# AlbrechtL/welle.io

Measured on AMD Instinct MI355X. Metric: DAB Mode-I ensembles/s (x real-time), higher is better.
Workload: dtype f32 (FFT/demap) + u16 (Viterbi metrics) + u8 (GF(256))

## Files before the change

### welle.io_amd/csrc/dabphy_fused.hip

```cpp
#include "dabphy_internal.h"
#include "soft_layout.h"

namespace {

bool step_table(const std::vector<map_t>& m, int nsteps, int n_in, int rows, bool skew, std::vector<MscStep>& st, int& n_windows, int& why)
{
    const int PITCH = MSC_ROW_PITCH, SLOT = rows * MSC_ROW_PITCH, ZERO = 2 * SLOT;
    constexpr int PADDING = 6;
    st.assign((size_t)nsteps + PADDING, MscStep{0, 0});
    std::vector<int> wlo((size_t)nsteps, -1), whi((size_t)nsteps, -1);
    for (int q = 0; q < nsteps; q++) {
        uint32_t off[4];
        for (int j = 0; j < 4; j++) {
            const int u = map_index(m[4 * q + j]);
            if (u < 0) { off[j] = (uint32_t)ZERO; continue; }
            const int w = u >> 4, col = u & 15;
            off[j] = (uint32_t)((w & 1) * SLOT + (skew ? layout::tdi_row(col) : 0) * PITCH + col);
            if (wlo[q] < 0) wlo[q] = w;
            whi[q] = w;
        }
        st[q].off01 = off[0] | (off[1] << 16); st[q].off23 = off[2] | (off[3] << 16);
    }
    for (int q = nsteps; q < nsteps + PADDING; q++) st[(size_t)q].off01 = st[(size_t)q].off23 = (uint32_t)ZERO | ((uint32_t)ZERO << 16);
    n_windows = (n_in + 15) / 16;
    std::vector<int> low_after((size_t)nsteps, n_windows);
    for (int q = nsteps - 2, low = n_windows; q >= 0; q--) { if (wlo[q + 1] >= 0) low = wlo[q + 1]; low_after[q] = low; }
    int seen = 1, prev_low = 0;
    std::vector<int> load_step((size_t)n_windows + 2, -10);
    bool ok = nsteps % 6 == 0; why = ok ? 0 : 8;
    for (int q = 0; q < nsteps; q++) {
        if (whi[q] > seen) {
            st[q].off01 |= MSC_FIRST_USE; seen = whi[q];
            if (q - 1 - load_step[seen] < 2) { ok = false; why |= 1; }
        }
        if (whi[q] >= 0 && whi[q] - wlo[q] > 1) { ok = false; why |= 2; }
        if (low_after[q] > prev_low) {
            if (low_after[q] != prev_low + 1 && low_after[q] < n_windows) { ok = false; why |= 4; }
            prev_low = low_after[q];
            if (prev_low + 1 < n_windows) { st[q].off01 |= MSC_LOAD_NEXT; load_step[prev_low + 1] = q; }
        }
    }
    return ok;
}

}

extern "C" {

size_t soft_ens_stride(const dabphy_handle* h)
{
    return ((size_t)h->cfg.max_frames + 5 + 1) * SOFT_PER_FRAME;
}

int fused_class_tables(dabphy_handle* h, const dabphy_protection& prot, bool fic, DevBuf (&steps)[FUSED_VARIANTS], int (&n_windows)[FUSED_VARIANTS])
{
    const std::vector<map_t> m = depuncture_map(&prot);
    const int nsteps = prot.nbits + 6, n_in = protection_input_bits(&prot);
    for (int v = 0; v < FUSED_VARIANTS; v++) {
        std::vector<MscStep> st; int nw = 0, why = 0;
        const bool ok = step_table(m, nsteps, n_in, FUSED_ROWS[v], !fic, st, nw, why);
        if (!ok && debug_env("DABPHY_DEBUG")) fprintf(stderr, "dabphy: class nbits %d: no fused decode (window schedule, reason %d)\n", prot.nbits, why);
        n_windows[v] = ok ? nw : 0;
        int r;
        if ((r = ensure(h, steps[v], st.size() * sizeof(MscStep)))) return r;
        HIPCHK(h, hipMemcpy(steps[v].p, st.data(), st.size() * sizeof(MscStep), hipMemcpyHostToDevice));
    }
    return DABPHY_OK;
}

int dabphy_test_fused_windows(const dabphy_protection* prot, int32_t n_windows[FUSED_VARIANTS])
{
    if (!prot || !n_windows || !protection_valid(prot) || prot->nbits > PRBS_MAX_BITS) return DABPHY_ERR_INVALID;
    dabphy_protection pf; protection_fic(&pf);
    const bool fic = !memcmp(prot, &pf, sizeof pf);
    const std::vector<map_t> m = depuncture_map(prot);
    for (int v = 0; v < FUSED_VARIANTS; v++) {
        std::vector<MscStep> st; int nw = 0, why = 0;
        n_windows[v] = step_table(m, prot->nbits + 6, protection_input_bits(prot), FUSED_ROWS[v], !fic, st, nw, why) ? nw : 0;
    }
    return DABPHY_OK;
}

}

namespace {
bool sp_kernel_takes(int nsteps) { return nsteps % 6 == 0 && nsteps <= SP_MAXSTEPS[SP_VARIANTS - 1]; }
bool sp_wanted(const dabphy_handle* h, uint64_t n_cw) { return h->fused_msc && h->cfg.decode_shape != 1 && (h->cfg.decode_shape >= 2 || (h->sp_max_codewords > 0 && n_cw <= h->sp_max_codewords)); }
struct Draft {
    uint32_t F = 0; bool want_fic = false; int v = 0;
    uint64_t total_cw = 0; bool use_sp = false;
    std::vector<FusedClass> cls; std::vector<int> idx; bool fic_in = false; size_t max_steps = 0;
    std::vector<uint32_t> work, item_off; uint64_t item_rows = 0;
    bool sp_two = false, tb_split = false, dec_by_item = false; int n_slots = 0; size_t slot_cells = 0, dec_cells = 0;
};

void choose_shape(const dabphy_handle* h, Draft& D)
{
    const bool fic = D.want_fic && h->fused_fic;
    D.total_cw = (uint64_t)h->cfg.n_ensembles * D.F * 4 * (fic ? 1 : 0);
    size_t longest = fic ? 774 : 0; bool takes = true;
    for (auto& c : h->classes) { D.total_cw += (uint64_t)4 * D.F * c.pairs.size(); longest = std::max(longest, (size_t)c.prot.nbits + 6); takes = takes && sp_kernel_takes(c.prot.nbits + 6); }
    const bool scratch_below_a_gib = D.total_cw * (uint64_t)hist_cells(longest, false) * sizeof(uint2) <= ((uint64_t)1 << 30);
    D.use_sp = takes && sp_wanted(h, D.total_cw) && (h->cfg.decode_shape >= 2 || scratch_below_a_gib);
}
void admit_classes(const dabphy_handle* h, Draft& D)
{
    const int nseg = (FUSED_ROWS[D.v] - 64) / 15, F = (int)D.F;
    auto reach_ok = [&](int n_ens_spanned) { return (uint64_t)n_ens_spanned * soft_ens_stride(h) <= 0xffffffffull; };
    auto ens_span = [&](const std::vector<MscPair>& pr) {
        int span = 1;
        for (size_t p = 0; p < pr.size(); p++) span = std::max(span, pr[std::min(pr.size() - 1, p + (size_t)nseg - 1)].ens - pr[p].ens + 1);
        return span;
    };
    for (size_t i = 0; i < h->classes.size(); i++) {
        const auto& c = h->classes[i];
        if (h->fused_msc && (D.use_sp || (c.n_windows[D.v] > 0 && reach_ok(ens_span(c.pairs))))) { D.cls.push_back(msc_fused_class(c, D.F, D.v)); D.idx.push_back((int)i); }
    }
    D.fic_in = D.want_fic && h->fused_fic && (D.use_sp || (h->fic_windows[D.v] > 0 && reach_ok((16 + F - 1) / F + 1)));
    if (D.fic_in) D.cls.push_back(fic_fused_class(h, h->s_fib.as<uint8_t>(), (int)(h->cfg.n_ensembles * D.F * 4), D.v));
    for (const FusedClass& fc : D.cls) D.max_steps = std::max(D.max_steps, (size_t)fc.nsteps);
}
int build_work_list(dabphy_handle* h, Draft& D)
{
    if (D.cls.size() > WORK_MAX_CLASSES) { h->err = "more than 255 protection classes"; return DABPHY_ERR_INVALID; }
    struct Item { int nsteps, ci, n_groups; }; std::vector<Item> items;
    for (size_t ci = 0; ci < D.cls.size(); ci++) items.push_back({D.cls[ci].nsteps, (int)ci, (D.cls[ci].n_cw + 63) / 64});
    std::stable_sort(items.begin(), items.end(), [](const Item& a, const Item& b) { return a.nsteps > b.nsteps; });
    for (const Item& it : items) {
        if (it.n_groups > (int)WORK_MAX_GROUPS) { h->err = "class too large for the fused decode's work list"; return DABPHY_ERR_INVALID; }
        for (int g = 0; g < it.n_groups; g++) { D.work.push_back(work_item((uint32_t)it.ci, (uint32_t)g)); D.item_off.push_back((uint32_t)D.item_rows); D.item_rows += (uint64_t)it.nsteps; }
    }
    return DABPHY_OK;
}
void lay_out_scratch(const dabphy_handle* h, Draft& D)
{
    const int slots = fused_wave_slots(D.v);
    D.sp_two = D.use_sp && sp_two_for(h, D.total_cw);
    D.n_slots = D.use_sp ? (int)D.work.size() * (D.sp_two ? 32 : 64) : (int)std::min<size_t>(D.work.size(), (size_t)slots);
    D.slot_cells = D.use_sp ? hist_cells(D.max_steps, D.sp_two) : D.max_steps * 64;
    D.tb_split = h->tb_split && !D.use_sp && D.item_rows < 0xffffffffull && !D.work.empty();
    D.dec_by_item = !D.use_sp && (D.tb_split || debug_env("DABPHY_FORCE_DEC_BY_ITEM") || D.item_rows < (uint64_t)D.n_slots * D.max_steps) && D.item_rows < 0xffffffffull;
    D.dec_cells = D.dec_by_item ? (size_t)D.item_rows * 64 : (size_t)D.n_slots * D.slot_cells;
}
int reserve_buffers(dabphy_handle* h, const Draft& D)
{
    int r;
    if (D.work.empty()) return DABPHY_OK;
    if ((r = ensure(h, h->vdec, D.dec_cells * sizeof(uint2))) || (D.dec_by_item && (r = ensure(h, h->fused_dec_off, D.item_off.size() * sizeof(uint32_t))))) return r;
    if (D.tb_split && (r = ensure(h, h->fused_done, (D.work.size() + 2) * sizeof(uint32_t)))) return r;
    if (D.tb_split && !h->tb_stream && ((r = new_stream(h, &h->tb_stream)) || (r = new_event(h, &h->ev_tb_fork)) || (r = new_event(h, &h->ev_tb_join)))) return r;
    if ((r = ensure(h, h->fused_cls, D.cls.size() * sizeof(FusedClass))) || (r = ensure(h, h->fused_work, D.work.size() * sizeof(uint32_t)))) return r;
    return h->d_fused_next ? DABPHY_OK : device_block(h, &h->d_fused_next, 1);
}
int upload_changed(dabphy_handle* h, const Draft& D)
{
    auto& P = h->fplan;
    const bool in_place = P.valid && P.buf_gen == h->buf_gen;
    const bool same_cls = in_place && table_holds(P.host_cls, D.cls);
    const bool same_work = in_place && table_holds(P.host_work, D.work) && P.dec_by_item == D.dec_by_item;
    if (P.valid && (!same_cls || !same_work)) HIPCHK(h, hipStreamSynchronize(h->stream));
    int r = same_cls ? 0 : upload_kept(h, h->fused_cls, P.host_cls, D.cls);
    if (!r && !same_work) r = upload_kept(h, h->fused_work, P.host_work, D.work);
    if (!r && !same_work && D.dec_by_item) r = upload_kept(h, h->fused_dec_off, P.host_dec_off, D.item_off);
    return r;
}
void keep_plan(dabphy_handle* h, const Draft& D)
{
    auto& P = h->fplan;
    if (debug_env("DABPHY_DEBUG")) fprintf(stderr, "dabphy: decode plan for %u frames per call: %s, %zu of %zu classes%s, %zu groups, %d work-groups, decision scratch %s\n", D.F, D.use_sp ? (D.sp_two ? "state-parallel, two code words per wavefront" : "state-parallel") : "lane-per-code-word", D.idx.size(), h->classes.size(), D.fic_in ? " + FIC" : "", D.work.size(), D.n_slots, D.dec_by_item ? "per group" : "per work-group");
    P.valid = true; P.F = D.F; P.want_fic = D.want_fic; P.fic_in = D.fic_in; P.variant = D.v; P.n_slots = D.n_slots; P.class_idx = D.idx; P.buf_gen = h->buf_gen;
    P.use_sp = D.use_sp; P.sp_variant = sp_variant_for((int)D.max_steps); P.sp_two = D.sp_two; P.dec_by_item = D.dec_by_item; P.tb_split = h->tb_split;
    FusedArgs& a = P.args; a = FusedArgs{};
    a.soft = h->s_soft.as<int8_t>(); a.ens_stride = soft_ens_stride(h); a.soft_ring = (int)h->cfg.max_frames + 5; a.n_ens = (int)h->cfg.n_ensembles; a.n_frames = (int)D.F;
    a.cls = h->fused_cls.as<FusedClass>(); a.work = h->fused_work.as<uint32_t>(); a.n_work = (uint32_t)D.work.size(); a.next = h->d_fused_next;
    a.dec = h->vdec.as<uint2>(); a.dec_slot_cells = D.slot_cells; a.prbs_words = h->d_prbs_words;
    a.dec_off = D.dec_by_item ? h->fused_dec_off.as<uint32_t>() : nullptr;
    if (D.tb_split) { a.done = h->fused_done.as<uint32_t>(); a.next_tb = a.done + D.work.size(); }
    a.sp2_warm = (int)h->sp2_tb_warm; a.sp2_resident = (int)h->sp2_tb_resident;
}
}

extern "C" {
int fused_plan(dabphy_handle* h, uint32_t F, bool want_fic)
{
    const auto& P = h->fplan;
    if (P.valid && P.F == F && P.want_fic == want_fic && P.buf_gen == h->buf_gen && P.tb_split == h->tb_split) return DABPHY_OK;
    Draft D; D.F = F; D.want_fic = want_fic; D.v = 4 * (int)F >= FUSED_MIN_CIFS[0] ? 0 : 4 * (int)F >= FUSED_MIN_CIFS[1] ? 1 : 2; int r;
    choose_shape(h, D);
    admit_classes(h, D);
    if ((r = build_work_list(h, D))) return r;
    lay_out_scratch(h, D);
    if ((r = reserve_buffers(h, D)) || (r = upload_changed(h, D))) return r;
    keep_plan(h, D);
    return DABPHY_OK;
}
void launch_plan(const dabphy_handle* h, hipStream_t s)
{
    const auto& P = h->fplan;
    if (P.use_sp) { launch_sp(P.args, P.sp_two, P.sp_variant, s); return; }
    const FusedSplit split{h->tb_no_walkers ? nullptr : h->tb_stream, h->ev_tb_fork, h->ev_tb_join};
    launch_viterbi_fused(P.args, P.variant, P.n_slots, s, P.args.done ? &split : nullptr);
}
// ... 65 lines not shown
```

### welle.io_amd/csrc/dabphy_kernels.h

```cpp
#pragma once
#include "dabphy_common.h"
#include "decode_work.h"

namespace dabphy {

struct RxState {
    int64_t pos;
    int64_t frame_no;
    int32_t local_phase;
    int32_t coarse;
    int32_t fine;
    int32_t synced;
    float s_level;
    int32_t lost;
    int32_t n_exact_sums;
    int32_t hist_count, hist_head;
    int32_t hist_dropped;
    int32_t n_relock_inexact;
    int32_t attempts;
    int32_t first_lock_attempts;
    int32_t n_wide_frames;
    int32_t n_chain_frames;
    int32_t calm_frames;
    int32_t acq_phase;
// ... 31 lines not shown
static_assert(sizeof(FrameDesc) == 80, "FrameDesc layout");

struct SyncArgs {
    Tables tab;
    const cf32* iq; size_t iq_stride; int64_t ring;
    int64_t n_valid;
    int loop;
    RxState* state; const DecState* dec; FrameDesc* desc; int n_ens, n_frames, frame;
    int fft_placement, disable_coarse, freqsync;
    float* cir;
    FrameDesc* hist; int hist_cap;
    float level_max;
    const int32_t* redo_from;
    int32_t* redo_out; int32_t* any_redo;
    int32_t* any_chain;
    int skip_wide;
    int last_round;
};

struct DemodArgs {
    Tables tab;
    const cf32* iq; size_t iq_stride; int64_t ring;
    const FrameDesc* desc; int n_frames;
    int chunk_len;
    int mix;
    int8_t* soft; int soft_ring;
    size_t soft_ens_stride;
    cf32* con;
    float* prs_mag;
    unsigned long long* osc_stats;
    int frame_first, frame_count, chunk_count;
};

struct SnrArgs {
    DecState* state; const FrameDesc* desc; int n_ens, n_frames;
    const float* prs_mag; float* snr_out;
};

struct VitClass {
    int nbits;
    int nsteps;
    int n_cw;
    int n_groups;
    int g_begin, g_end;
    uint32_t* sym;
    uint2* dec;
    uint8_t* out;
    int dedisperse;
};

struct VitArgs { VitClass c; const uint32_t* prbs_words; };

struct FicGatherArgs {
    const int8_t* soft; int soft_ring; size_t frame_stride;
    size_t soft_ens_stride;
    const FrameDesc* desc; int n_ens, n_frames;
    const map_t* map;
    VitClass c;
    int frame_sel;
};

struct MscPair {
    int32_t ens;
    int32_t start_bit;
    int64_t cif0;
    int32_t idx;
    int32_t pad_;
};
static_assert(sizeof(MscPair) == 24, "MscPair layout");
void launch_pair_cif0(MscPair* pairs, int n_pairs, const FrameDesc* desc, int n_frames, hipStream_t s);

struct MscGatherArgs {
    const int8_t* soft; int soft_ring; const RxState* state; int n_ens, n_frames;
    size_t soft_ens_stride;
    const map_t* map;
    const MscPair* pairs;
    const int32_t* tiles;
    int n_pairs;
    const FrameDesc* desc;
    VitClass c;
};

struct MscStep { uint32_t off01, off23; };
constexpr int MSC_ROW_PITCH = 20;
constexpr int FUSED_VARIANTS = 3;
constexpr int FUSED_ROWS[FUSED_VARIANTS] = {96, 144, 324};
constexpr int FUSED_MIN_CIFS[FUSED_VARIANTS] = {64, 16, 4};
constexpr uint32_t MSC_FIRST_USE = 1u << 15, MSC_LOAD_NEXT = 1u << 31, MSC_OFF_MASK = 0x7fffu;
struct FusedClass {
    const MscStep* steps;
    const MscPair* pairs;
    const map_t* map;
    uint8_t* out;
    int32_t nsteps, nbits, n_windows, n_cw, n_pairs, kind, dedisperse, reserved_;
};
static_assert(sizeof(FusedClass) == 64, "FusedClass layout");
struct FusedArgs {
    const int8_t* soft; size_t ens_stride; int soft_ring; int n_ens, n_frames;
    const FrameDesc* desc;
    const FusedClass* cls;
    const uint32_t* work; uint32_t n_work;
    uint32_t* next;
    uint2* dec; size_t dec_slot_cells;
    const uint32_t* dec_off;
    const uint32_t* prbs_words;
    uint32_t* done; uint32_t* next_tb;
    int fic_frame_sel;
    size_t fic_frame_stride;
    const int8_t* lin_in; size_t lin_stride;
    int sp2_warm;
    int sp2_resident;
};
struct FusedSplit { hipStream_t tb_stream; hipEvent_t fork, join; };
void launch_viterbi_fused(const FusedArgs& a, int variant, int n_slots, hipStream_t s, const FusedSplit* split = nullptr);
int fused_wave_slots(int variant);
constexpr int SP_VARIANTS = 3;
constexpr int SP_MAXSTEPS[SP_VARIANTS] = {1542, 3078, 9222};
void launch_viterbi_sp(const FusedArgs& a, int lds_variant, hipStream_t s);
void launch_selftest_pair_exchange(unsigned* out, hipStream_t s);
constexpr int SP2_VARIANTS = 2;
void launch_viterbi_sp2(const FusedArgs& a, int lds_variant, hipStream_t s);
void launch_selftest_half_exchange(unsigned* out, hipStream_t s);

struct BerArgs { FusedArgs f; const uint32_t* first; uint2* out; };
struct BerTotalsArgs { const uint2* counts; const uint32_t* slots; uint32_t n; uint64_t* totals; };
void launch_chanber(const BerArgs& a, hipStream_t s);
void launch_chanber_totals(const BerTotalsArgs& a, int n_slots, hipStream_t s);

struct CrcArgs {
    const uint8_t* fib;
    uint8_t* ok;
    DecState* state; const FrameDesc* desc; int n_ens, n_frames;
    int disable_coarse;
    int frame_first, frame_count;
    int32_t* any_effective;
    int frame_sel;
};

struct LinGatherArgs {
    const int8_t* in; size_t in_stride;
    const map_t* map;
    VitClass c;
};

struct NullArgs {
    Tables tab; const cf32* iq; size_t iq_stride; int64_t ring;
    const FrameDesc* desc; int n_frames;
    cf32* out;
};
void launch_null_symbols(const NullArgs& a, int n_ens, hipStream_t s);

constexpr int TII_MAX_LIKELY = 9;
constexpr int TII_SLOTS = 32;
struct TiiSlot { int32_t cp1, num, cycle, pad; unsigned long long acc[TII_NERR]; };
struct TiiEvent { int32_t frame, comb, pattern, delay_samples; float error; };
struct TiiArgs {
    Tables tab; const cf32* iq; size_t iq_stride; int64_t ring;
    const FrameDesc* desc; int n_ens, n_frames;
    const cf32* rot; const int32_t* rank; const uint8_t* pattern;
    float* abs_err;
    int32_t* likely;
    TiiSlot* state;
    TiiEvent* events; int32_t* n_events; int max_events;
    int32_t* overflow;
};
void launch_tii(const TiiArgs& a, hipStream_t s);

struct IngestArgs {
    const uint8_t* raw; size_t raw_stride;
    cf32* iq; size_t iq_stride; uint64_t ring, w, n;
    int format;
};
void launch_ingest(const IngestArgs& a, int n_ens, hipStream_t s);
__device__ __forceinline__ cf32 ingest_sample(const uint8_t* __restrict__ src, uint64_t i, int format)
{
    cf32 v;
    if (format == 1) {
// ... 156 lines not shown
```

### welle.io_amd/csrc/k_viterbi.hip

```cpp
#include "dabphy_kernels.h"
#include <cstdlib>
#include <dabphy_wave_ops.h>
#include "viterbi_acs.h"
#include "soft_layout.h"

namespace dabphy {

__device__ __forceinline__ uint32_t pack_step(uint32_t s0, uint32_t s1, uint32_t s2, uint32_t s3)
{
    return ((s0 + s3 - 254u) & 0xffffu) | (((s1 - 127u) & 0xffu) << 16) | ((s2 - 127u) << 24);
}
__device__ __forceinline__ uint32_t pack_step_word(uint32_t w) { return pack_step(w & 0xff, (w >> 8) & 0xff, (w >> 16) & 0xff, w >> 24); }
template <int F>
__device__ __forceinline__ uint2 step_from_word(uint32_t (&M)[32], uint32_t w, uint32_t ones)
{
    return acs::step<F>(M, (int)(int16_t)(w & 0xffffu), (int)(int8_t)((w >> 16) & 0xffu), (int)w >> 24, ones);
}

template <typename LoadDec>
__device__ __forceinline__ void traceback(LoadDec&& load_dec, int nbits, uint32_t* __restrict__ out, bool live,
                                          int dedisperse, const uint32_t* __restrict__ prbs_words)
{
    uint32_t J = 0, outw = 0;
    uint32_t rho = (uint32_t)acs::dec_rot((nbits - 1) % 6);
// ... 128 lines not shown
    if (t == 0) {
        int nrows = 0;
        for (int l = 0; l < 64;) {
            int e = l;
            while (e + 1 < 64 && s_pair[e + 1] == s_pair[l] && s_c[e + 1] == s_c[e] + 1) e++;
            const int need = (e - l) + 16;
            if (s_pair[l] < 0) { for (int k = l; k <= e; k++) s_rowbase[k] = -1; l = e + 1; continue; }
            if (nrows + need > GT_MAXROWS) { nrows = -1; break; }
            const MscPair pp = A.pairs[s_pair[l]];
            const long long pbase = (long long)pp.ens * (long long)ens_stride + pp.start_bit;
            for (int k = 0; k < need; k++) {
                const long long c_src = s_c[l] - 16 + k;
                long long src = -1;
                if (c_src >= 0) src = pbase + (long long)layout::cif_row_bytes(c_src, A.soft_ring);
                s_rowsrc[nrows + k] = src;
            }
            for (int k = l; k <= e; k++) s_rowbase[k] = nrows + (k - l);
            nrows += need;
            l = e + 1;
        }
        s_nrows = nrows;
    }
    __syncthreads();
    const int nrows = s_nrows;
    const int rowbase = s_rowbase[lane];

    if (nrows < 0) {
        for (int s = wave; s < nsteps; s += 4) {
            uint32_t word = 0;
#pragma unroll
            for (int j = 0; j < 4; j++) {
                const int u = map_index(A.map[4 * s + j]);
                int v = 0;
                if (u >= 0 && live) {
                    const long long c_src = c_glob - 16 + layout::tdi_row(u & 15);
                    if (c_src >= 0) v = A.soft[ens_base + layout::cif_row_bytes(c_src, A.soft_ring) + u];
                }
                v += 127; v = v < 0 ? 0 : v; v = v > 255 ? 255 : v;
                word |= (uint32_t)v << (8 * j);
            }
            dst[(size_t)s * 64] = pack_step_word(word);
        }
        return;
    }

    const int8_t* tile8 = reinterpret_cast<const int8_t*>(tile);
    __shared__ __attribute__((aligned(16))) int s_map[4 * GT_STEPS];
    for (int s0 = 0, ti = 0; s0 < nsteps; s0 += GT_STEPS, ti++) {
        const int u_lo = A.tiles[2 * ti], ndw = A.tiles[2 * ti + 1];
        const int s1 = (s0 + GT_STEPS < nsteps) ? s0 + GT_STEPS : nsteps;
        if (t < 4 * (s1 - s0)) {
            const int u = map_index(A.map[4 * s0 + t]);
            s_map[t] = (u >= 0) ? (layout::tdi_row(u & 15) * (GT_PITCHW * 4) + (u - u_lo)) : -1;
        }
        for (int row = wave; row < nrows; row += 4) {
            const long long src = s_rowsrc[row];
            if (lane < ndw) {
                if (src >= 0) lds_dma4(A.soft + src + u_lo + 4 * lane, &tile[row * GT_PITCHW]);
                else tile[row * GT_PITCHW + lane] = 0u;
            }
        }
        lds_dma_wait();
        __syncthreads();
        const int rb = rowbase * (GT_PITCHW * 4);
        auto pick = [&](int off) { int v = (off >= 0 && rowbase >= 0) ? (int)tile8[rb + off] : 0; v += 127; return v < 0 ? 0 : v; };
        int s = s0 + wave;
        for (; s + 4 < s1; s += 8) {
            const int4 ma = *reinterpret_cast<const int4*>(&s_map[4 * (s - s0)]);
            const int4 mb = *reinterpret_cast<const int4*>(&s_map[4 * (s + 4 - s0)]);
            const int a0 = pick(ma.x), a1 = pick(ma.y), a2 = pick(ma.z), a3 = pick(ma.w);
            const int b0 = pick(mb.x), b1 = pick(mb.y), b2 = pick(mb.z), b3 = pick(mb.w);
            dst[(size_t)s * 64] = pack_step(a0, a1, a2, a3);
            dst[(size_t)(s + 4) * 64] = pack_step(b0, b1, b2, b3);
        }
        if (s < s1) {
            const int4 ma = *reinterpret_cast<const int4*>(&s_map[4 * (s - s0)]);
            const int a0 = pick(ma.x), a1 = pick(ma.y), a2 = pick(ma.z), a3 = pick(ma.w);
            dst[(size_t)s * 64] = pack_step(a0, a1, a2, a3);
        }
        __syncthreads();
    }
}

constexpr int FM_PITCH = MSC_ROW_PITCH;
constexpr int FM_REQ_ROWS = 12;
template <int ROWS> struct FmGeom {
    static constexpr int SLOT = ROWS * FM_PITCH;
    static constexpr int ZERO = 2 * SLOT;
    static constexpr int ROWPTR = 3 * SLOT;
    static constexpr int LDS = ROWPTR + ROWS * 4;
    static constexpr int NREQ = ROWS / FM_REQ_ROWS;
    static_assert(ROWS % FM_REQ_ROWS == 0 && 3 * SLOT + 64 * FM_PITCH <= (int)MSC_OFF_MASK, "window ring geometry");
};
#ifndef FM_DEC_STORE_AUX
#define FM_DEC_STORE_AUX 0
#endif
#ifndef FM_DEC_LOAD_AUX
#define FM_DEC_LOAD_AUX 2
#endif

#ifndef VITM_OCC
#define VITM_OCC 5
#endif
__device__ __forceinline__ void tb_publish(const FusedArgs& A, uint32_t item, int lane)
{
    __builtin_amdgcn_fence(__ATOMIC_RELEASE, "agent");
    lds_dma_wait();
    (void)lane; __hip_atomic_store(A.done + item, 1u, __ATOMIC_RELAXED, __HIP_MEMORY_SCOPE_AGENT);
}
template <bool LEAN>
__device__ __forceinline__ void tb_consume(const FusedArgs& A, int lane)
{
    const DABPHY_CONST_AS uint32_t* const dec_off = as_constant(A.dec_off);
    const DABPHY_CONST_AS FusedClass* const classes = as_constant(A.cls);
    const DABPHY_CONST_AS uint32_t* const work = as_constant(A.work);
    const uint32_t lane8 = (uint32_t)lane * 8u;
#pragma unroll 1
    for (;;) {
        uint32_t item = 0;
        if (lane == 0) item = atomicAdd(A.next_tb, 1u);
        item = (uint32_t)uniform_i32(__shfl((int)item, 0));
        if (item >= A.n_work) break;
        uint32_t polls = 0;
        for (;;) {
            uint32_t f = 0;
            if (lane == 0) f = atomicAdd(A.done + item, 0u);
            f = (uint32_t)uniform_i32(__shfl((int)f, 0));
            if (f) break;
            __builtin_amdgcn_s_sleep(127);
            if (++polls > (1u << 19)) { if (lane == 0) atomicAdd(A.done + A.n_work + 1, 1u); break; }
        }
        __builtin_amdgcn_fence(__ATOMIC_ACQUIRE, "agent");
        const uint32_t wk = work[item];
        const DABPHY_CONST_AS FusedClass& C = classes[work_class(wk)];
        const int g = (int)work_group(wk);
        const int nbits = C.nbits, n_cw = C.n_cw;
        const BufRsrc dec_rs = buf_rsrc(A.dec + (size_t)dec_off[item] * 64);
        const int cw_out = g * 64 + lane;
        uint32_t* const out = reinterpret_cast<uint32_t*>(C.out) + (size_t)cw_out * (nbits / 32);
        const bool live = cw_out < n_cw;
        if constexpr (!LEAN) {
            traceback([&](int st) { return buf_load_b64<FM_DEC_LOAD_AUX>(dec_rs, lane8, (uint32_t)st * 512u); }, nbits, out, live, C.dedisperse, A.prbs_words);
        } else {
            uint32_t J = 0, outw = 0;
            uint32_t rho = (uint32_t)acs::dec_rot((nbits - 1) % 6);
#pragma unroll 1
            for (int n = nbits - 1; n >= 0; n -= 8) {
                uint2 dq[8];
#pragma unroll
                for (int k = 0; k < 8; k++) dq[k] = buf_load_b64<FM_DEC_LOAD_AUX>(dec_rs, lane8, (uint32_t)(n - k + 6) * 512u);
#pragma unroll
                for (int k = 0; k < 8; k++) { acs::back(dq[k], J, outw, rho); rho = rho == 5 ? 0 : rho + 1; }
                if (((n - 7) & 31) == 0) {
                    const int wi = (n - 7) >> 5;
                    const uint32_t word = acs::back_word(outw);
                    if (live) out[wi] = C.dedisperse ? word ^ A.prbs_words[wi] : word;
                }
            }
        }
    }
}

template <int ROWS, int OCC, bool SPLIT>
__global__ void __launch_bounds__(64, OCC) k_viterbi_fused(FusedArgs A)
{
  using G = FmGeom<ROWS>;
  __shared__ __attribute__((aligned(16))) uint8_t lds[G::LDS];
  const int lane = threadIdx.x;
  const int F = A.n_frames, R = 4 * F;
  const uint32_t lane8 = (uint32_t)lane * 8u;
  const DABPHY_CONST_AS uint32_t* const dec_off = as_constant(A.dec_off);
  const DABPHY_CONST_AS FusedClass* const classes = as_constant(A.cls);
  const DABPHY_CONST_AS uint32_t* const work = as_constant(A.work);
  uint32_t* const rowptr = reinterpret_cast<uint32_t*>(lds + G::ROWPTR);
#pragma unroll 1
  for (;;) {
    uint32_t item = 0;
    if (lane == 0) item = atomicAdd(A.next, 1u);
    item = (uint32_t)uniform_i32(__shfl((int)item, 0));
    if (item >= A.n_work) break;
    const uint32_t wk = work[item];
    const BufRsrc dec_rs = buf_rsrc(A.dec + (A.dec_off ? (size_t)dec_off[item] * 64 : (size_t)blockIdx.x * A.dec_slot_cells));
    const DABPHY_CONST_AS FusedClass& C = classes[work_class(wk)];
    const int g = (int)work_group(wk);
    const int nsteps = C.nsteps, nbits = C.nbits, n_cw = C.n_cw, n_windows = C.n_windows;
    const long long cw0 = (long long)g * 64;
    const int cw = (int)cw0 + lane;
    const uint32_t zero16 = (uint32_t)(((size_t)A.soft_ring * SOFT_PER_FRAME) >> 4);
    __syncthreads();
    for (int i = lane; i < G::ROWPTR / 16; i += 64) reinterpret_cast<uint4*>(lds)[i] = make_uint4(0, 0, 0, 0);
    int rb, nrows, pb0;
    if (C.kind == 0) {
        const MscPair* __restrict__ pairs = C.pairs;
        const int pair0 = (int)(cw0 / R), r0 = (int)(cw0 - (long long)pair0 * R);
        const int n0 = R - r0;
        const long long cw_last = cw0 + 63 < n_cw ? cw0 + 63 : (long long)n_cw - 1;
        const int nseg = (int)(cw_last / R) - pair0 + 1;
        nrows = 64 + 15 * nseg;
        pb0 = pairs[pair0].ens;
        int seg = cw / R - pair0; if (seg > nseg - 1) seg = nseg - 1;
        rb = lane + 15 * seg;
        for (int row = lane; row < ROWS; row += 64) {
            uint32_t src = zero16;
            if (row < nrows) {
                int j = 0, idx = row;
                if (row >= n0 + 15) { const int q = row - (n0 + 15); j = 1 + q / (R + 15); idx = q - (j - 1) * (R + 15); }
                const int pr = pair0 + j;
                if (j == 0 || (long long)pr * R < n_cw) {
                    const MscPair pp = pairs[pr];
                    const int pb = pp.ens;
                    const long long c_src = 4 * A.desc[(size_t)pb * F].frame_no + (j == 0 ? r0 : 0) - 16 + idx;
                    if (c_src >= 0)
                        src = (uint32_t)(((size_t)(pb - pb0) * A.ens_stride + (size_t)pp.start_bit + layout::cif_row_bytes(c_src, A.soft_ring)) >> 4);
                }
            }
            rowptr[row] = src;
        }
    } else {
        nrows = 64; rb = lane;
        pb0 = layout::fic_frame_of((int)cw0, F, 0) / F;
        for (int row = lane; row < ROWS; row += 64) {
            uint32_t src = zero16;
            const int cwr = (int)cw0 + row;
            if (row < 64 && cwr < n_cw) {
                const int bf = layout::fic_frame_of(cwr, F, 0), b = bf / F;
                const FrameDesc& d = A.desc[bf];
                if (d.valid == 1)
                    src = (uint32_t)(((size_t)(b - pb0) * A.ens_stride + layout::fic_cw_bytes(d.frame_no, A.soft_ring, SOFT_PER_FRAME, cwr)) >> 4);
            }
            rowptr[row] = src;
        }
    }
    __syncthreads();
    const BufRsrc soft_rs = buf_rsrc_4g(A.soft + (size_t)uniform_i32(pb0) * A.ens_stride);
    const int nreq = uniform_i32((nrows + FM_REQ_ROWS - 1) / FM_REQ_ROWS);
    auto load_window = [&](int w) {
        uint8_t* slot = lds + (w & 1) * G::SLOT;
        const uint32_t l = opaque_vgpr((uint32_t)lane);
        const uint32_t r5 = (l * 205u) >> 10, q5 = l - 5u * r5;
        if (q5 < 4u && l < 5u * FM_REQ_ROWS) {
            if constexpr (G::NREQ == 8) {
                uint32_t src[8];
#pragma unroll
                for (int k = 0; k < 8; k++) src[k] = rowptr[FM_REQ_ROWS * k + r5];
#pragma unroll
                for (int k = 0; k < 8; k++) buf_dma4(soft_rs, (src[k] << 4) + 4u * q5, 16u * (uint32_t)w, slot + FM_REQ_ROWS * FM_PITCH * k);
            } else {
#pragma unroll 1
                for (int k0 = 0; k0 < nreq; k0 += 3) {
                    uint32_t src[3];
#pragma unroll
                    for (int k = 0; k < 3; k++) src[k] = rowptr[FM_REQ_ROWS * (k0 + k) + r5];
#pragma unroll
                    for (int k = 0; k < 3; k++) if (k0 + k < nreq) buf_dma4(soft_rs, (src[k] << 4) + 4u * q5, 16u * (uint32_t)w, slot + FM_REQ_ROWS * FM_PITCH * (k0 + k));
                }
            }
        }
    };
    load_window(0);
    if (n_windows > 1) load_window(1);

    const uint32_t ones = opaque_sgpr(0x01010101u);
    uint32_t M[32];
    acs::init(M);
#ifdef FM_EXP_BROADCAST
    const uint32_t lane_base = 0u; (void)rb;
#else
    const uint32_t lane_base = (uint32_t)rb * (uint32_t)FM_PITCH;
#endif
    const int8_t* lds_c = reinterpret_cast<const int8_t*>(lds);
    auto fetch = [&](const MscStep& d, int (&y)[4]) {
#ifdef FM_EXP_NOLDS
        y[0] = (int)(d.off01 & 127) - 60; y[1] = (int)(d.off23 & 127) - 61; y[2] = lane - 30; y[3] = 5; return;
#endif
        y[0] = lds_c[lane_base + (d.off01 & MSC_OFF_MASK)]; y[1] = lds_c[lane_base + ((d.off01 >> 16) & MSC_OFF_MASK)];
        y[2] = lds_c[lane_base + (d.off23 & 0xffffu)]; y[3] = lds_c[lane_base + (d.off23 >> 16)];
    };
    lds_dma_wait();
    int cur[4];
    int next_window = 2;
    const DABPHY_CONST_AS MscStep* steps = as_constant(C.steps);
    auto desc_at = [&](int i) { MscStep d; d.off01 = steps[i].off01; d.off23 = steps[i].off23; return d; };
    auto one_step = [&](auto fc, int s, const MscStep& d_cur, const MscStep& d_next, auto&& after_wait) {
        constexpr int FL = decltype(fc)::value;
        int x0 = cur[0] + cur[3], v1 = cur[1], v2 = cur[2];
        asm volatile("" : "+v"(x0), "+v"(v1), "+v"(v2));
        after_wait();
#ifndef FM_EXP_NODMA
        if (d_cur.off01 & MSC_LOAD_NEXT) { wave_converge(); load_window(next_window); next_window++; }
#endif
        const uint2 dd = acs::step<FL>(M, x0, v1, v2, ones);
#ifdef FM_EXP_NOSTORE
        if (dd.x == 0x12345u && dd.y == 0x777u) buf_store_b64<FM_DEC_STORE_AUX>(dec_rs, lane8, (uint32_t)s * 512u, dd);
#else
        buf_store_b64<FM_DEC_STORE_AUX>(dec_rs, lane8, (uint32_t)s * 512u, dd);
#endif
#ifndef FM_EXP_NOWAIT
        if (d_next.off01 & MSC_FIRST_USE) lds_dma_wait_but<2>();
#endif
        fetch(d_next, cur);
    };
    auto nothing = []() {};
    MscStep d0 = desc_at(0), d1 = desc_at(1), d2 = desc_at(2), d3 = desc_at(3), d4 = desc_at(4), d5 = desc_at(5);
    fetch(d0, cur);
    int since_renorm = 0;
    for (int s = 0; s < nsteps; s += 6) {
        MscStep ea, eb;
        one_step(std::integral_constant<int, 0>{}, s, d0, d1, [&]() { ea = desc_at(s + 6); eb = desc_at(s + 7); });
        one_step(std::integral_constant<int, 1>{}, s + 1, d1, d2, nothing);
        d0 = ea; d1 = eb;
        one_step(std::integral_constant<int, 2>{}, s + 2, d2, d3, [&]() { ea = desc_at(s + 8); eb = desc_at(s + 9); });
        one_step(std::integral_constant<int, 3>{}, s + 3, d3, d4, nothing);
        d2 = ea; d3 = eb;
        one_step(std::integral_constant<int, 4>{}, s + 4, d4, d5, [&]() { ea = desc_at(s + 10); eb = desc_at(s + 11); });
        one_step(std::integral_constant<int, 5>{}, s + 5, d5, d0, nothing);
        d4 = ea; d5 = eb;
        if (++since_renorm == acs::RENORM_BLOCKS) { acs::renorm(M); since_renorm = 0; }
    }
    lds_dma_wait();

#ifndef FM_EXP_NOTRACE
    if constexpr (SPLIT) {
        tb_publish(A, item, lane);
    } else {
        const int cw_out = g * 64 + lane;
        traceback([&](int st) { return buf_load_b64<FM_DEC_LOAD_AUX>(dec_rs, lane8, (uint32_t)st * 512u); }, nbits,
                  reinterpret_cast<uint32_t*>(C.out) + (size_t)cw_out * (nbits / 32), cw_out < n_cw, C.dedisperse, A.prbs_words);
    }
#endif
  }
#ifndef FM_EXP_NOTRACE
  if constexpr (SPLIT) tb_consume<false>(A, lane);
#endif
}

__global__ void __launch_bounds__(64) __attribute__((amdgpu_num_vgpr(32))) k_traceback_fused(FusedArgs A)
{
    tb_consume<true>(A, threadIdx.x);
}

static int device_simds()
{
    static int n_simd = 0;
    if (!n_simd) {
        int dev = 0; hipDeviceProp_t p;
        n_simd = (hipGetDevice(&dev) == hipSuccess && hipGetDeviceProperties(&p, dev) == hipSuccess) ? 4 * p.multiProcessorCount : 1024;
    }
    return n_simd;
}
constexpr int FUSED_OCC[FUSED_VARIANTS] = {VITM_OCC, 4, 1};
int fused_wave_slots(int variant)
{
    int occ = FUSED_OCC[variant];
#ifdef DABPHY_EXPERIMENTS
    { const char* e = getenv("DABPHY_VITM_SLOTS"); if (e && atoi(e) > 0) occ = atoi(e); }
    { const char* e = getenv("DABPHY_VITM_SLOTS_PCT"); if (e && atoi(e) > 0 && atoi(e) <= 100) return (int)((long long)occ * device_simds() * atoi(e) / 100); }
#endif
    return occ * device_simds();
}
void launch_viterbi_fused(const FusedArgs& a, int variant, int n_slots, hipStream_t s, const FusedSplit* split)
{
    if (a.n_work == 0 || n_slots <= 0) return;
    hipError_t e = hipMemsetAsync(a.next, 0, sizeof(uint32_t), s); (void)e;
    if (a.done && split) {
        e = hipMemsetAsync(a.done, 0, ((size_t)a.n_work + 2) * sizeof(uint32_t), s);
        if (split->tb_stream) { e = hipEventRecord(split->fork, s); e = hipStreamWaitEvent(split->tb_stream, split->fork, 0); }
        if (variant == 0) hipLaunchKernelGGL((k_viterbi_fused<FUSED_ROWS[0], FUSED_OCC[0], true>), dim3(n_slots), dim3(64), 0, s, a);
        else if (variant == 1) hipLaunchKernelGGL((k_viterbi_fused<FUSED_ROWS[1], FUSED_OCC[1], true>), dim3(n_slots), dim3(64), 0, s, a);
        else hipLaunchKernelGGL((k_viterbi_fused<FUSED_ROWS[2], FUSED_OCC[2], true>), dim3(n_slots), dim3(64), 0, s, a);
        if (split->tb_stream) {
            const int n_tb = std::min<int>((int)a.n_work, device_simds());
            hipLaunchKernelGGL(k_traceback_fused, dim3(n_tb), dim3(64), 0, split->tb_stream, a);
            e = hipEventRecord(split->join, split->tb_stream);
            e = hipStreamWaitEvent(s, split->join, 0);
        }
        return;
    }
    if (variant == 0) hipLaunchKernelGGL((k_viterbi_fused<FUSED_ROWS[0], FUSED_OCC[0], false>), dim3(n_slots), dim3(64), 0, s, a);
    else if (variant == 1) hipLaunchKernelGGL((k_viterbi_fused<FUSED_ROWS[1], FUSED_OCC[1], false>), dim3(n_slots), dim3(64), 0, s, a);
    else hipLaunchKernelGGL((k_viterbi_fused<FUSED_ROWS[2], FUSED_OCC[2], false>), dim3(n_slots), dim3(64), 0, s, a);
}
// ... 120 lines not shown
```

Measured before the change: 78680.

## Widen fused Viterbi soft-bit windows and adapt DMA wait depth per class

The fused decode's LDS window ring now has a geometry per variant. The 96-row variant uses 32-column windows (pitch 36), the others keep 16. The erased-bit zero row is replaced by a fixed erased column, which shrinks LDS so more waves can fit. The step table also computes a per-class wait depth (6, 4 or 2 outstanding DMAs), so first-use waits block less. In exchange the kernel gains runtime branches on wait depth, a different DMA request layout with an overlapping last request, and a larger window per load.

```diff
diff --git a/welle.io_amd/csrc/dabphy_fused.hip b/welle.io_amd/csrc/dabphy_fused.hip
--- a/welle.io_amd/csrc/dabphy_fused.hip
+++ b/welle.io_amd/csrc/dabphy_fused.hip
@@ -1,49 +1,6 @@
 #include "dabphy_internal.h"
 #include "soft_layout.h"
-
-namespace {
-
-bool step_table(const std::vector<map_t>& m, int nsteps, int n_in, int rows, bool skew, std::vector<MscStep>& st, int& n_windows, int& why)
-{
-    const int PITCH = MSC_ROW_PITCH, SLOT = rows * MSC_ROW_PITCH, ZERO = 2 * SLOT;
-    constexpr int PADDING = 6;
-    st.assign((size_t)nsteps + PADDING, MscStep{0, 0});
-    std::vector<int> wlo((size_t)nsteps, -1), whi((size_t)nsteps, -1);
-    for (int q = 0; q < nsteps; q++) {
-        uint32_t off[4];
-        for (int j = 0; j < 4; j++) {
-            const int u = map_index(m[4 * q + j]);
-            if (u < 0) { off[j] = (uint32_t)ZERO; continue; }
-            const int w = u >> 4, col = u & 15;
-            off[j] = (uint32_t)((w & 1) * SLOT + (skew ? layout::tdi_row(col) : 0) * PITCH + col);
-            if (wlo[q] < 0) wlo[q] = w;
-            whi[q] = w;
-        }
-        st[q].off01 = off[0] | (off[1] << 16); st[q].off23 = off[2] | (off[3] << 16);
-    }
-    for (int q = nsteps; q < nsteps + PADDING; q++) st[(size_t)q].off01 = st[(size_t)q].off23 = (uint32_t)ZERO | ((uint32_t)ZERO << 16);
-    n_windows = (n_in + 15) / 16;
-    std::vector<int> low_after((size_t)nsteps, n_windows);
-    for (int q = nsteps - 2, low = n_windows; q >= 0; q--) { if (wlo[q + 1] >= 0) low = wlo[q + 1]; low_after[q] = low; }
-    int seen = 1, prev_low = 0;
-    std::vector<int> load_step((size_t)n_windows + 2, -10);
-    bool ok = nsteps % 6 == 0; why = ok ? 0 : 8;
-    for (int q = 0; q < nsteps; q++) {
-        if (whi[q] > seen) {
-            st[q].off01 |= MSC_FIRST_USE; seen = whi[q];
-            if (q - 1 - load_step[seen] < 2) { ok = false; why |= 1; }
-        }
-        if (whi[q] >= 0 && whi[q] - wlo[q] > 1) { ok = false; why |= 2; }
-        if (low_after[q] > prev_low) {
-            if (low_after[q] != prev_low + 1 && low_after[q] < n_windows) { ok = false; why |= 4; }
-            prev_low = low_after[q];
-            if (prev_low + 1 < n_windows) { st[q].off01 |= MSC_LOAD_NEXT; load_step[prev_low + 1] = q; }
-        }
-    }
-    return ok;
-}
-
-}
+#include "window_table.h"
 
 extern "C" {
 
@@ -52,18 +9,20 @@
     return ((size_t)h->cfg.max_frames + 5 + 1) * SOFT_PER_FRAME;
 }
 
+static StepTable class_step_table(const dabphy_protection& prot, bool fic, int v)
+{
+    return step_table(depuncture_map(&prot), prot.nbits + 6, protection_input_bits(&prot), fused_geom(v), !fic);
+}
+
 int fused_class_tables(dabphy_handle* h, const dabphy_protection& prot, bool fic, DevBuf (&steps)[FUSED_VARIANTS], int (&n_windows)[FUSED_VARIANTS])
 {
-    const std::vector<map_t> m = depuncture_map(&prot);
-    const int nsteps = prot.nbits + 6, n_in = protection_input_bits(&prot);
     for (int v = 0; v < FUSED_VARIANTS; v++) {
-        std::vector<MscStep> st; int nw = 0, why = 0;
-        const bool ok = step_table(m, nsteps, n_in, FUSED_ROWS[v], !fic, st, nw, why);
-        if (!ok && debug_env("DABPHY_DEBUG")) fprintf(stderr, "dabphy: class nbits %d: no fused decode (window schedule, reason %d)\n", prot.nbits, why);
-        n_windows[v] = ok ? nw : 0;
+        const StepTable T = class_step_table(prot, fic, v);
+        if (!T.ok && debug_env("DABPHY_DEBUG")) fprintf(stderr, "dabphy: class nbits %d: no fused decode (window schedule, reason %d)\n", prot.nbits, T.why);
+        n_windows[v] = T.ok ? T.n_windows : 0;
         int r;
-        if ((r = ensure(h, steps[v], st.size() * sizeof(MscStep)))) return r;
-        HIPCHK(h, hipMemcpy(steps[v].p, st.data(), st.size() * sizeof(MscStep), hipMemcpyHostToDevice));
+        if ((r = ensure(h, steps[v], T.st.size() * sizeof(MscStep)))) return r;
+        HIPCHK(h, hipMemcpy(steps[v].p, T.st.data(), T.st.size() * sizeof(MscStep), hipMemcpyHostToDevice));
     }
     return DABPHY_OK;
 }
@@ -73,11 +32,7 @@
     if (!prot || !n_windows || !protection_valid(prot) || prot->nbits > PRBS_MAX_BITS) return DABPHY_ERR_INVALID;
     dabphy_protection pf; protection_fic(&pf);
     const bool fic = !memcmp(prot, &pf, sizeof pf);
-    const std::vector<map_t> m = depuncture_map(prot);
-    for (int v = 0; v < FUSED_VARIANTS; v++) {
-        std::vector<MscStep> st; int nw = 0, why = 0;
-        n_windows[v] = step_table(m, prot->nbits + 6, protection_input_bits(prot), FUSED_ROWS[v], !fic, st, nw, why) ? nw : 0;
-    }
+    for (int v = 0; v < FUSED_VARIANTS; v++) n_windows[v] = class_step_table(*prot, fic, v).ok ? (protection_input_bits(prot) + 15) / 16 : 0;
     return DABPHY_OK;
 }
 
@@ -114,10 +69,11 @@
     };
     for (size_t i = 0; i < h->classes.size(); i++) {
         const auto& c = h->classes[i];
-        if (h->fused_msc && (D.use_sp || (c.n_windows[D.v] > 0 && reach_ok(ens_span(c.pairs))))) { D.cls.push_back(msc_fused_class(c, D.F, D.v)); D.idx.push_back((int)i); }
+        if (h->fused_msc && (D.use_sp || (c.n_windows[D.v] > 0 && reach_ok(ens_span(c.pairs))))) { D.cls.push_back(msc_fused_class(c, D.F, D.v)); D.idx.push_back((int)i); if (!D.use_sp) D.cls.back().wait_depth = class_step_table(c.prot, false, D.v).wait_depth; }
     }
     D.fic_in = D.want_fic && h->fused_fic && (D.use_sp || (h->fic_windows[D.v] > 0 && reach_ok((16 + F - 1) / F + 1)));
     if (D.fic_in) D.cls.push_back(fic_fused_class(h, h->s_fib.as<uint8_t>(), (int)(h->cfg.n_ensembles * D.F * 4), D.v));
+    if (D.fic_in && !D.use_sp) { dabphy_protection pf; protection_fic(&pf); D.cls.back().wait_depth = class_step_table(pf, true, D.v).wait_depth; }
     for (const FusedClass& fc : D.cls) D.max_steps = std::max(D.max_steps, (size_t)fc.nsteps);
 }
 int build_work_list(dabphy_handle* h, Draft& D)
diff --git a/welle.io_amd/csrc/dabphy_kernels.h b/welle.io_amd/csrc/dabphy_kernels.h
--- a/welle.io_amd/csrc/dabphy_kernels.h
+++ b/welle.io_amd/csrc/dabphy_kernels.h
@@ -137,17 +137,35 @@
 };
 
 struct MscStep { uint32_t off01, off23; };
-constexpr int MSC_ROW_PITCH = 20;
 constexpr int FUSED_VARIANTS = 3;
 constexpr int FUSED_ROWS[FUSED_VARIANTS] = {96, 144, 324};
 constexpr int FUSED_MIN_CIFS[FUSED_VARIANTS] = {64, 16, 4};
+constexpr int FUSED_WIN[FUSED_VARIANTS] = {32, 16, 16};
 constexpr uint32_t MSC_FIRST_USE = 1u << 15, MSC_LOAD_NEXT = 1u << 31, MSC_OFF_MASK = 0x7fffu;
+struct WinGeom {
+    int rows, win;
+    constexpr int pitch() const { return win + 4; }
+    constexpr int slot() const { return rows * pitch(); }
+    constexpr int erased() const { return win; }
+    constexpr int rowptr() const { return 2 * slot(); }
+    constexpr int lds() const { return rowptr() + rows * 4; }
+    constexpr int dwords() const { return pitch() / 4; }
+    constexpr int req_rows() const { return 64 / dwords(); }
+    constexpr int n_req() const { return (rows + req_rows() - 1) / req_rows(); }
+    constexpr bool fits() const { return 2 * slot() + 64 * pitch() <= (int)MSC_OFF_MASK && win % 16 == 0 && dwords() % 2 == 1 && req_rows() <= rows; }
+};
+constexpr WinGeom fused_geom(int variant) { return WinGeom{FUSED_ROWS[variant], FUSED_WIN[variant]}; }
+constexpr int fused_variant_of_rows(int rows) { return rows == FUSED_ROWS[0] ? 0 : rows == FUSED_ROWS[1] ? 1 : 2; }
+static_assert(fused_geom(0).fits() && fused_geom(1).fits() && fused_geom(2).fits(), "window ring geometry: offsets of 15 bits, odd dword pitch");
+static_assert(fused_geom(0).lds() == 7296, "96 rows: twenty waves per compute unit in 160 KiB");
+constexpr int FUSED_WAIT_DEPTHS[3] = {6, 4, 2};
 struct FusedClass {
     const MscStep* steps;
     const MscPair* pairs;
     const map_t* map;
     uint8_t* out;
-    int32_t nsteps, nbits, n_windows, n_cw, n_pairs, kind, dedisperse, reserved_;
+    int32_t nsteps, nbits, n_windows, n_cw, n_pairs, kind, dedisperse;
+    int32_t wait_depth;
 };
 static_assert(sizeof(FusedClass) == 64, "FusedClass layout");
 struct FusedArgs {
diff --git a/welle.io_amd/csrc/k_viterbi.hip b/welle.io_amd/csrc/k_viterbi.hip
--- a/welle.io_amd/csrc/k_viterbi.hip
+++ b/welle.io_amd/csrc/k_viterbi.hip
@@ -234,15 +234,19 @@
     }
 }
 
-constexpr int FM_PITCH = MSC_ROW_PITCH;
-constexpr int FM_REQ_ROWS = 12;
 template <int ROWS> struct FmGeom {
-    static constexpr int SLOT = ROWS * FM_PITCH;
-    static constexpr int ZERO = 2 * SLOT;
-    static constexpr int ROWPTR = 3 * SLOT;
-    static constexpr int LDS = ROWPTR + ROWS * 4;
-    static constexpr int NREQ = ROWS / FM_REQ_ROWS;
-    static_assert(ROWS % FM_REQ_ROWS == 0 && 3 * SLOT + 64 * FM_PITCH <= (int)MSC_OFF_MASK, "window ring geometry");
+    static constexpr WinGeom G = fused_geom(fused_variant_of_rows(ROWS));
+    static constexpr int WIN = G.win;
+    static constexpr int PITCH = G.pitch();
+    static constexpr int SLOT = G.slot();
+    static constexpr int ROWPTR = G.rowptr();
+    static constexpr int LDS = G.lds();
+    static constexpr int DW = G.dwords();
+    static constexpr int REQ_ROWS = G.req_rows();
+    static constexpr int NREQ = G.n_req();
+    static constexpr uint32_t DIV_MUL = DW == 5 ? 205u : 57u, DIV_SH = DW == 5 ? 10u : 9u;
+    static constexpr bool div_exact() { for (uint32_t l = 0; l < 64; l++) if (((l * DIV_MUL) >> DIV_SH) != l / (uint32_t)DW) return false; return true; }
+    static_assert(ROWS == G.rows && (DW == 5 || DW == 9) && div_exact() && REQ_ROWS * DW <= 64 && G.fits(), "window ring geometry");
 };
 #ifndef FM_DEC_STORE_AUX
 #define FM_DEC_STORE_AUX 0
@@ -335,7 +339,7 @@
     const BufRsrc dec_rs = buf_rsrc(A.dec + (A.dec_off ? (size_t)dec_off[item] * 64 : (size_t)blockIdx.x * A.dec_slot_cells));
     const DABPHY_CONST_AS FusedClass& C = classes[work_class(wk)];
     const int g = (int)work_group(wk);
-    const int nsteps = C.nsteps, nbits = C.nbits, n_cw = C.n_cw, n_windows = C.n_windows;
+    const int nsteps = C.nsteps, nbits = C.nbits, n_cw = C.n_cw, n_windows = C.n_windows, wait_depth = C.wait_depth;
     const long long cw0 = (long long)g * 64;
     const int cw = (int)cw0 + lane;
     const uint32_t zero16 = (uint32_t)(((size_t)A.soft_ring * SOFT_PER_FRAME) >> 4);
@@ -385,26 +389,28 @@
     }
     __syncthreads();
     const BufRsrc soft_rs = buf_rsrc_4g(A.soft + (size_t)uniform_i32(pb0) * A.ens_stride);
-    const int nreq = uniform_i32((nrows + FM_REQ_ROWS - 1) / FM_REQ_ROWS);
+    const int nreq = uniform_i32((nrows + G::REQ_ROWS - 1) / G::REQ_ROWS);
     auto load_window = [&](int w) {
         uint8_t* slot = lds + (w & 1) * G::SLOT;
         const uint32_t l = opaque_vgpr((uint32_t)lane);
-        const uint32_t r5 = (l * 205u) >> 10, q5 = l - 5u * r5;
-        if (q5 < 4u && l < 5u * FM_REQ_ROWS) {
-            if constexpr (G::NREQ == 8) {
-                uint32_t src[8];
-#pragma unroll
-                for (int k = 0; k < 8; k++) src[k] = rowptr[FM_REQ_ROWS * k + r5];
-#pragma unroll
-                for (int k = 0; k < 8; k++) buf_dma4(soft_rs, (src[k] << 4) + 4u * q5, 16u * (uint32_t)w, slot + FM_REQ_ROWS * FM_PITCH * k);
+        const uint32_t r = (l * G::DIV_MUL) >> G::DIV_SH, q = l - (uint32_t)G::DW * r;
+        auto row0 = [](int k) { return k * G::REQ_ROWS + G::REQ_ROWS <= ROWS ? k * G::REQ_ROWS : ROWS - G::REQ_ROWS; };
+        if (q < (uint32_t)G::DW - 1u && l < (uint32_t)(G::DW * G::REQ_ROWS)) {
+            if constexpr (ROWS == FUSED_ROWS[0]) {
+                uint32_t src[G::NREQ];
+#pragma unroll
+                for (int k = 0; k < G::NREQ; k++) src[k] = rowptr[row0(k) + r];
+#pragma unroll
+                for (int k = 0; k < G::NREQ; k++) buf_dma4(soft_rs, (src[k] << 4) + 4u * q, (uint32_t)G::WIN * (uint32_t)w, slot + G::PITCH * row0(k));
             } else {
+                static_assert(G::NREQ % 3 == 0 && ROWS % G::REQ_ROWS == 0, "requests in threes");
 #pragma unroll 1
                 for (int k0 = 0; k0 < nreq; k0 += 3) {
                     uint32_t src[3];
 #pragma unroll
-                    for (int k = 0; k < 3; k++) src[k] = rowptr[FM_REQ_ROWS * (k0 + k) + r5];
-#pragma unroll
-                    for (int k = 0; k < 3; k++) if (k0 + k < nreq) buf_dma4(soft_rs, (src[k] << 4) + 4u * q5, 16u * (uint32_t)w, slot + FM_REQ_ROWS * FM_PITCH * (k0 + k));
+                    for (int k = 0; k < 3; k++) src[k] = rowptr[G::REQ_ROWS * (k0 + k) + r];
+#pragma unroll
+                    for (int k = 0; k < 3; k++) if (k0 + k < nreq) buf_dma4(soft_rs, (src[k] << 4) + 4u * q, (uint32_t)G::WIN * (uint32_t)w, slot + G::REQ_ROWS * G::PITCH * (k0 + k));
                 }
             }
         }
@@ -418,7 +424,7 @@
 #ifdef FM_EXP_BROADCAST
     const uint32_t lane_base = 0u; (void)rb;
 #else
-    const uint32_t lane_base = (uint32_t)rb * (uint32_t)FM_PITCH;
+    const uint32_t lane_base = (uint32_t)rb * (uint32_t)G::PITCH;
 #endif
     const int8_t* lds_c = reinterpret_cast<const int8_t*>(lds);
     auto fetch = [&](const MscStep& d, int (&y)[4]) {
@@ -448,7 +454,9 @@
         buf_store_b64<FM_DEC_STORE_AUX>(dec_rs, lane8, (uint32_t)s * 512u, dd);
 #endif
 #ifndef FM_EXP_NOWAIT
-        if (d_next.off01 & MSC_FIRST_USE) lds_dma_wait_but<2>();
+        if (d_next.off01 & MSC_FIRST_USE) {
+            if (wait_depth >= 6) lds_dma_wait_but<6>(); else if (wait_depth >= 4) lds_dma_wait_but<4>(); else lds_dma_wait_but<2>();
+        }
 #endif
         fetch(d_next, cur);
     };
diff --git a/welle.io_amd/csrc/window_table.h b/welle.io_amd/csrc/window_table.h
--- /dev/null
+++ b/welle.io_amd/csrc/window_table.h
@@ -0,0 +1,63 @@
+#pragma once
+#include "dabphy_kernels.h"
+#include "soft_layout.h"
+#include <algorithm>
+#include <vector>
+
+namespace dabphy {
+
+constexpr int STEP_TABLE_PADDING = 6;
+
+struct StepTable {
+    std::vector<MscStep> st;
+    int n_windows = 0;
+    int wait_depth = 0;
+    int why = 0;
+    bool ok = false;
+};
+
+inline StepTable step_table(const std::vector<map_t>& m, int nsteps, int n_in, WinGeom G, bool skew)
+{
+    StepTable T;
+    const int WIN = G.win, PITCH = G.pitch(), SLOT = G.slot();
+    const uint32_t ERASED = (uint32_t)G.erased();
+    T.st.assign((size_t)nsteps + STEP_TABLE_PADDING, MscStep{0, 0});
+    std::vector<int> wlo((size_t)nsteps, -1), whi((size_t)nsteps, -1);
+    for (int q = 0; q < nsteps; q++) {
+        uint32_t off[4];
+        for (int j = 0; j < 4; j++) {
+            const int u = map_index(m[4 * q + j]);
+            if (u < 0) { off[j] = ERASED; continue; }
+            const int w = u / WIN, col = u % WIN;
+            off[j] = (uint32_t)((w & 1) * SLOT + (skew ? layout::tdi_row(col & 15) : 0) * PITCH + col);
+            if (wlo[q] < 0) wlo[q] = w;
+            whi[q] = w;
+        }
+        T.st[q].off01 = off[0] | (off[1] << 16); T.st[q].off23 = off[2] | (off[3] << 16);
+    }
+    for (int q = nsteps; q < nsteps + STEP_TABLE_PADDING; q++) T.st[(size_t)q].off01 = T.st[(size_t)q].off23 = ERASED | (ERASED << 16);
+    const int n_windows = T.n_windows = (n_in + WIN - 1) / WIN;
+    std::vector<int> low_after((size_t)nsteps, n_windows);
+    for (int q = nsteps - 2, low = n_windows; q >= 0; q--) { if (wlo[q + 1] >= 0) low = wlo[q + 1]; low_after[q] = low; }
+    int seen = 1, prev_low = 0, youngest = 1 << 30;
+    std::vector<int> load_step((size_t)n_windows + 2, -(1 << 20));
+    bool ok = nsteps % 6 == 0; T.why = ok ? 0 : 8;
+    for (int q = 0; q < nsteps; q++) {
+        if (whi[q] > seen) {
+            T.st[q].off01 |= MSC_FIRST_USE; seen = whi[q];
+            youngest = std::min(youngest, q - 1 - load_step[seen]);
+        }
+        if (whi[q] >= 0 && whi[q] - wlo[q] > 1) { ok = false; T.why |= 2; }
+        if (low_after[q] > prev_low) {
+            if (low_after[q] != prev_low + 1 && low_after[q] < n_windows) { ok = false; T.why |= 4; }
+            prev_low = low_after[q];
+            if (prev_low + 1 < n_windows) { T.st[q].off01 |= MSC_LOAD_NEXT; load_step[prev_low + 1] = q; }
+        }
+    }
+    for (int d : FUSED_WAIT_DEPTHS) if (!T.wait_depth && youngest >= d) T.wait_depth = d;
+    if (!T.wait_depth) { ok = false; T.why |= 1; }
+    T.ok = ok;
+    return T;
+}
+
+}
```

Result: no change. 79030, median of 4 (+0.4%).
